# nubomedia/NUBOMEDIA-VCA

Hardware: AMD Instinct MI355X
Metric: 1080p frames/sec/node (NuboFaceDetector); achieved HBM GB/s vs peak (higher is better)
Workload: dtype i32 rect sums / f32 products / f64 stage sums (u8 pixels)

## Files before the change

nubomedia-vca_amd/csrc/api.cpp:

```cpp
#include "nvca_internal.h"
#include "plan.h"
#include "host_logic.h"
#include <cstdio>
#include <cstring>
#include <cmath>
#include <climits>
#include <algorithm>
#include <fstream>
#include <sstream>
#include <chrono>
#if defined(__SSE2__)
#include <emmintrin.h>
#endif
#include <stdexcept>
#include <new>
#include <thread>
#include <condition_variable>
#include <atomic>

using namespace nvca;

namespace nvca {

static bool alloc_log() { static const bool on = getenv("NVCA_ALLOC_LOG") != nullptr; return on; }
// ... 129 lines not shown
    t.pending.swap(later);
}
static void drain_timer(nvca_ctx *ctx)
{
    if (ctx->timer.pending.size() > 4096) drain_timer_now(ctx);
}

int api_catch(nvca_ctx *ctx) noexcept
{
    int code = NVCA_ERR_INTERNAL;
    const char *what = "unknown exception";
    char buf[160];
    try { throw; }
    catch (const std::bad_alloc &) { code = NVCA_ERR_NOMEM; what = "out of host memory (std::bad_alloc)"; }
    catch (const std::length_error &e) { code = NVCA_ERR_NOMEM; snprintf(buf, sizeof(buf), "container size limit exceeded (%s)", e.what()); what = buf; }
    catch (const std::exception &e) { snprintf(buf, sizeof(buf), "internal error: %s", e.what()); what = buf; }
    catch (...) { }
    if (ctx) {
        try { std::lock_guard<std::recursive_mutex> lk(ctx->mu); ctx->err.assign(what); } catch (...) { }
    }
    return code;
}

static Switches read_switches()
{
    Switches w;
    auto num = [](const char *name, int dflt) { const char *e = getenv(name); return e ? atoi(e) : dflt; };
    auto set = [](const char *name) { return getenv(name) != nullptr; };
    w.group_zero_copy = num("NVCA_GROUP_ZEROCOPY", 1) != 0;
    w.skip_cascade = set("NVCA_SKIP_CASCADE");
    w.host_group = set("NVCA_HOST_GROUP");
    w.band_map = num("NVCA_BAND_MAP", 0);
    w.band = num("NVCA_BAND", -1);
    w.host_profile = set("NVCA_HOST_PROFILE");
    w.sparse_ingest = num("NVCA_SPARSE_INGEST", 1) != 0;
    w.pyr_off = set("NVCA_PYR_OFF");
    if (set("NVCA_PART_STATS")) { const int n = num("NVCA_PART_STATS", 0); w.part_stats = n > 0 ? n : 8; }
    w.ingest_chunk = num("NVCA_INGEST_CHUNK", 8);
    w.stage_order = num("NVCA_STAGE_ORDER", 0) != 0;
    w.trk_fold = num("NVCA_TRK_FOLD", 1) != 0;
    w.spec_pairs = std::max(1, num("NVCA_SPEC_PAIRS", 1536));
    w.pair_max = num("NVCA_PAIR_MAX", 32);
    w.deep_stage = set("NVCA_DEEP_STAGE") ? std::max(1, num("NVCA_DEEP_STAGE", 0)) : 0;
    w.tiles = num("NVCA_TILES", 1) != 0;
    w.plan_debug = set("NVCA_PLAN_DEBUG");
    w.deep_lds = !set("NVCA_DEEP_LDS_OFF");
    w.trk_order = num("NVCA_TRK_ORDER", -1);
    w.host_threads = num("NVCA_HOST_THREADS", -1);
    w.two_lanes = num("NVCA_TWO_LANES", 1) != 0;
    w.roi = num("NVCA_ROI", 1) != 0;
    w.fb_dense = num("NVCA_FB_DENSE", 1) != 0;
    w.pre_cus = num("NVCA_PRE_CUS", 0);
    w.quiet = set("NVCA_QUIET");
    w.stamps_out = getenv("NVCA_STAMPS_OUT");
    return w;
}
const Switches &switches()
{
    static const Switches w = read_switches();
    return w;
}

static inline size_t round_up(size_t v, size_t a) { return (v + a - 1) / a * a; }
static inline int cv_round(double v)
{
    if (!(v > -2147483648.5 && v < 2147483647.5)) return INT_MIN;
// ... 271 lines not shown
    const size_t grp_stride = rec + 2;
    if (dev_group) {
        const void *old_gthr = rb.gthr.p;
        if (rb.grp.ensure((size_t)total * grp_stride * sizeof(int)) || rb.h_grp.ensure((size_t)total * grp_stride * sizeof(int)) ||
            rb.gthr.ensure((size_t)total * sizeof(int)) || rb.h_gthr.ensure((size_t)total * sizeof(int))) {
            ctx->set_error("device allocation failed for the grouping workspace"); return NVCA_ERR_NOMEM;
        }
        if (rb.gthr.p != old_gthr) rb.gthr_last.clear();
        job.d_grp = rb.grp.as<int>() + grp_stride * job.r0; job.h_grp = rb.h_grp.as<int>() + grp_stride * job.r0;
        if (rb.gthr_last.size() < (size_t)total) rb.gthr_last.resize(total, -1);
        if (memcmp(rb.gthr_last.data() + job.r0, group_thr, batch * sizeof(int)) != 0) {
            NVCA_HIP_CHECK(ctx, hipStreamSynchronize(ctx->cs()));
            memcpy(rb.h_gthr.as<int>() + job.r0, group_thr, batch * sizeof(int));
            NVCA_HIP_CHECK(ctx, hipMemcpyAsync(rb.gthr.as<int>() + job.r0, rb.h_gthr.as<int>() + job.r0, batch * sizeof(int), hipMemcpyHostToDevice, ctx->cs()));
            std::copy(group_thr, group_thr + batch, rb.gthr_last.begin() + job.r0);
        }
    }
    if (!dp.tasks.empty() && !skip_cascade) {
        CascadeArgs a;
        a.sum = ws.ln().sum.as<int>(); a.sqsum = ws.ln().sqsum.as<unsigned long long>();
        a.sum_slot = sum_slot; a.spitch = spitch;
        a.scales = dp.d_scales.as<ScaleRec>();
        a.stages = dp.d_stages.as<StageRec>(); a.strips = dp.d_strips.as<StripRec>(); a.pos = dp.d_pos.as<int>();
        a.order = dp.d_order.as<int>(); a.blocks_per_frame = dp.blocks_per_frame;
        a.tasks = dp.d_tasks.as<unsigned>(); a.ntasks = (int)dp.tasks.size();
        a.failbits = ws.ln().failbits.as<unsigned long long>(); a.vnf = ws.ln().vnf.as<double>();
        a.nstages = (int)dp.stages.size(); a.pair_policy = ctx->policy == NVCA_SUM_F32PAIR; a.stage_order = ctx->sw.stage_order ? 1 : 0; a.stage_hint = dp.d_stage_hint.as<int>(); a.stage_first = dp.d_stage_first.as<int>(); a.stage_thr = dp.d_stage_thr.as<float>(); a.spec_pairs = ctx->sw.spec_pairs; a.pair_max = std::min(32, std::max(0, ctx->sw.pair_max));
        a.deep_stage = dp.deep_stage; a.deep = ws.ln().deep.as<unsigned long long>(); a.deep_cap = deep_cap;
        a.hits = job.d_hits; a.hit_cap = cap;
        a.tiles = dp.d_tiles.as<TileRec>(); a.tile_order = dp.d_tile_order.as<int>();
        a.tile_blocks_per_frame = dp.tile_blocks_per_frame;
        a.tcoords = dp.d_tcoords.as<unsigned short>(); a.tile_lds = dp.tile_lds;
        a.nscales = (int)dp.scales.size(); a.key_sy = dp.key_sy; a.key_ss = dp.key_ss;
        a.bands = dp.d_bands.as<BandRec>(); a.band_order = dp.d_band_order.as<int>(); a.band_blocks_per_frame = dp.band_blocks_per_frame; a.batch = batch;
        { const int bm = ctx->sw.band_map; a.band_map = (bm > 0 && batch % (8 * bm) == 0) ? bm : 0; }
        a.deeprecs = dp.deeprecs.empty() ? nullptr : dp.d_deeprecs.as<DeepRec>(); a.deep_lds = dp.deep_lds;
        a.tilted = dp.needs_tilted ? ws.ln().tilted.as<int>() : nullptr;
        a.galpha = dp.tabs.empty() ? nullptr : dp.tabs[0]->d_galpha; a.gcls_first = dp.tabs.empty() ? nullptr : dp.tabs[0]->d_gcls_first;
        a.stump_based = dp.generic_stumps ? 1 : 0;
        if (dp.generic) {
            if (dp.needs_tilted && !a.tilted) { ctx->set_error("internal: tilted integral missing"); return NVCA_ERR_ARG; }
            { TimedLaunch t(ctx, NVCA_K_STAGE0); launch_generic(ctx->cs(), a, batch, 0); }
            { TimedLaunch t(ctx, NVCA_K_STRIP); launch_generic(ctx->cs(), a, batch, 1); }
        } else {
#ifdef NVCA_STAMPS
        {
            static DevBuf dbgbuf;
            a.dbg = nullptr;
            if (switches().stamps_out && !dbgbuf.ensure(64 * 16 * 64 * 8)) { a.dbg = dbgbuf.as<unsigned long long>(); (void)hipMemsetAsync(a.dbg, 0, 64 * 16 * 64 * 8, ctx->cs()); ctx->stamps = a.dbg; }
        }
#endif
        const int band_env = ctx->sw.band;
        const bool use_band = !dp.bands.empty() && (band_env >= 0 ? band_env != 0 : (long long)dp.bands.size() * batch >= 270 * kTilesPerCu);
        auto launch = [&](int which) {
            const int e = launch_cascade_sc(ctx->cs(), a, batch, which, ctx->lds_grant);
            if (e) ctx->set_error(std::string("hipFuncSetAttribute(MaxDynamicSharedMemorySize): ") + hipGetErrorString((hipError_t)e));
            return e;
        };
        if (!use_band) { TimedLaunch t(ctx, NVCA_K_STAGE0); if (launch(0)) return NVCA_ERR_HIP; }
        if (use_band) {
            TimedLaunch t(ctx, NVCA_K_BAND); if (launch(5)) return NVCA_ERR_HIP;
        } else {
            { TimedLaunch t(ctx, NVCA_K_TILE); if (launch(3)) return NVCA_ERR_HIP; }
            { TimedLaunch t(ctx, NVCA_K_STRIP); if (launch(1)) return NVCA_ERR_HIP; }
        }
        if (early_done) NVCA_HIP_CHECK(ctx, hipEventRecord(early_done, ctx->cs()));
        { TimedLaunch t(ctx, NVCA_K_DEEP); if (launch(2)) return NVCA_ERR_HIP; }
// ... 386 lines not shown
int nvca_ctx_set_hit_capacity(nvca_ctx *ctx, int cap)
try {
    if (!ctx || cap < 1 || cap > kMaxHitCap) return NVCA_ERR_ARG;
    ctx->hit_cap = cap;
    return NVCA_OK;
}
NVCA_API_CATCH(ctx)
int nvca_ctx_set_option(nvca_ctx *ctx, const char *name, int value)
try {
    NVCA_LOCK_OR_FAIL(ctx);
    if (!name) return NVCA_ERR_ARG;
    const std::string n(name);
    Switches &w = ctx->sw;
    bool replan = false;
    if (n == "band") w.band = value;
    else if (n == "band_map") w.band_map = value;
    else if (n == "group_zerocopy") w.group_zero_copy = value != 0;
    else if (n == "host_group") w.host_group = value != 0;
    else if (n == "skip_cascade") w.skip_cascade = value != 0;
    else if (n == "host_profile") w.host_profile = value != 0;
    else if (n == "sparse_ingest") w.sparse_ingest = value != 0;
    else if (n == "ingest_chunk") w.ingest_chunk = value;
    else if (n == "part_stats") w.part_stats = value;
    else if (n == "trk_order") w.trk_order = value;
    else if (n == "trk_fold") w.trk_fold = value != 0;
    else if (n == "quiet") w.quiet = value != 0;
    else if (n == "roi") w.roi = value != 0;
    else if (n == "fb_dense") w.fb_dense = value != 0;
    else if (n == "two_lanes") w.two_lanes = value != 0;
    else if (n == "host_threads") { w.host_threads = value; work_pool_destroy(ctx->pool); ctx->pool = nullptr; ctx->pool_tried = false; }
    else if (n == "pre_cus") w.pre_cus = value > 0 ? value : 0;
    else if (n == "plan_debug") w.plan_debug = value != 0;
    else if (n == "stage_order") w.stage_order = value != 0;
    else if (n == "spec_pairs") w.spec_pairs = value > 0 ? value : 1;
    else if (n == "pair_max") w.pair_max = value;
    else if (n == "pyr_off") { w.pyr_off = value != 0; replan = true; }
    else if (n == "tiles") { w.tiles = value != 0; replan = true; }
    else if (n == "deep_stage") { w.deep_stage = value > 0 ? value : 0; replan = true; }
    else if (n == "deep_lds") { w.deep_lds = value != 0; replan = true; }
    else { ctx->set_error("unknown option: " + n); return NVCA_ERR_ARG; }
    if (replan) {
        for (auto &kv : ctx->plans) if (kv.second->inflight) { ctx->set_error("a batch is in flight: collect it before changing a plan option"); return NVCA_ERR_ARG; }
        (void)hipSetDevice(ctx->device);
        NVCA_HIP_CHECK(ctx, hipDeviceSynchronize());
        ctx->plans.clear();
    }
    return NVCA_OK;
}
NVCA_API_CATCH(ctx)
int nvca_ctx_get_option(nvca_ctx *ctx, const char *name, int *value)
try {
    NVCA_LOCK_OR_FAIL(ctx);
    if (!name || !value) return NVCA_ERR_ARG;
    const std::string n(name);
    const Switches &w = ctx->sw;
    if (n == "band") *value = w.band;
    else if (n == "band_map") *value = w.band_map;
    else if (n == "group_zerocopy") *value = w.group_zero_copy;
    else if (n == "host_group") *value = w.host_group;
    else if (n == "skip_cascade") *value = w.skip_cascade;
    else if (n == "host_profile") *value = w.host_profile;
    else if (n == "sparse_ingest") *value = w.sparse_ingest;
    else if (n == "ingest_chunk") *value = w.ingest_chunk;
    else if (n == "part_stats") *value = w.part_stats;
    else if (n == "trk_order") *value = w.trk_order;
    else if (n == "trk_fold") *value = w.trk_fold;
    else if (n == "quiet") *value = w.quiet;
    else if (n == "roi") *value = w.roi;
    else if (n == "fb_dense") *value = w.fb_dense;
    else if (n == "two_lanes") *value = w.two_lanes;
    else if (n == "host_threads") *value = w.host_threads;
    else if (n == "pre_cus") *value = w.pre_cus;
    else if (n == "plan_debug") *value = w.plan_debug;
    else if (n == "stage_order") *value = w.stage_order;
    else if (n == "spec_pairs") *value = w.spec_pairs;
    else if (n == "pair_max") *value = w.pair_max;
    else if (n == "pyr_off") *value = w.pyr_off;
    else if (n == "tiles") *value = w.tiles;
    else if (n == "deep_stage") *value = w.deep_stage;
    else if (n == "deep_lds") *value = w.deep_lds;
    else { ctx->set_error("unknown option: " + n); return NVCA_ERR_ARG; }
    return NVCA_OK;
}
NVCA_API_CATCH(ctx)
int nvca_ctx_set_sum_policy(nvca_ctx *ctx, int policy)
try {
    if (!ctx || (policy != NVCA_SUM_F32PAIR && policy != NVCA_SUM_F64)) return NVCA_ERR_ARG;
    ctx->policy = policy;
    return NVCA_OK;
}
NVCA_API_CATCH(ctx)
int nvca_ctx_synchronize(nvca_ctx *ctx)
try {
    NVCA_LOCK_OR_FAIL(ctx);
    if (!ctx) return NVCA_ERR_ARG;
    NVCA_HIP_CHECK(ctx, hipStreamSynchronize(ctx->cs()));
    NVCA_HIP_CHECK(ctx, hipStreamSynchronize(ctx->lane_streams[kFaceLane2]));
    NVCA_HIP_CHECK(ctx, hipStreamSynchronize(ctx->lane_streams[kTrackerLane]));
#ifdef NVCA_STAMPS
    if (ctx->stamps && switches().stamps_out) {
        std::vector<unsigned long long> h(64 * 16 * 64);
        (void)hipMemcpy(h.data(), ctx->stamps, h.size() * 8, hipMemcpyDeviceToHost);
        if (FILE *f = fopen(switches().stamps_out, "wb")) { fwrite(h.data(), 8, h.size(), f); fclose(f); }
    }
    if (switches().stamps_out) roi_stamps_dump((std::string(switches().stamps_out) + ".roi.txt").c_str());
#endif
    return NVCA_OK;
// ... 1950 lines not shown
```

nubomedia-vca_amd/csrc/kernels_cascade.hip:

```cpp
#include "nvca_internal.h"

namespace nvca {

typedef const __attribute__((address_space(4))) TStumpRec CTStumpRec;
template <class T> __device__ __forceinline__ T load_const(const T *p)
{
    static_assert(sizeof(T) % 4 == 0, "dword records only");
    typedef const __attribute__((address_space(4))) int CInt;
    CInt *q = (CInt *)p;
    T r;
    int *d = (int *)&r;
#pragma unroll
    for (int i = 0; i < (int)(sizeof(T) / 4); i++) d[i] = q[i];
    return r;
}

__device__ __forceinline__ int ldsum(const int *__restrict__ sum, unsigned idx) { return sum[idx]; }

__device__ __forceinline__ double window_sqsum(const unsigned *__restrict__ sql, const uint8_t *__restrict__ sqh, bool lo_only,
                                               unsigned e0, unsigned e1, unsigned e2, unsigned e3)
{
    if (lo_only) return (double)(unsigned)(sql[e0] - sql[e1] - sql[e2] + sql[e3]);
    const unsigned long long q0 = ((unsigned long long)sqh[e0] << 32) | sql[e0], q1 = ((unsigned long long)sqh[e1] << 32) | sql[e1];
    const unsigned long long q2 = ((unsigned long long)sqh[e2] << 32) | sql[e2], q3 = ((unsigned long long)sqh[e3] << 32) | sql[e3];
// ... 480 lines not shown
    const int c0 = lds_u16(cm + (xx & 0xffffu)), c1 = lds_u16(cm + (xx >> 16));
    const int r0 = lds_u16(rm + (yy & 0xffffu)), r1 = lds_u16(rm + (yy >> 16));
    return lds_sample(r0, c0) - lds_sample(r0, c1) - lds_sample(r1, c0) + lds_sample(r1, c1);
}
__device__ __forceinline__ double lane_vote(unsigned cm, unsigned rm, double vnf, const LRec &f, int pair_policy)
{
    const int s0 = lane_rect(cm, rm, (unsigned)f.a.x, (unsigned)f.a.y);
    const int s1 = lane_rect(cm, rm, (unsigned)f.a.z, (unsigned)f.a.w);
    const double t = (double)__int_as_float(f.c.y) * vnf;
    const float p0 = (float)s0 * __int_as_float(f.b.z), p1 = (float)s1 * __int_as_float(f.b.w);
    double v = (double)p0;
    v += (double)p1;
    if (f.b.x) v += (double)((float)lane_rect(cm, rm, (unsigned)f.b.x, (unsigned)f.b.y) * __int_as_float(f.c.x));
    else if (pair_policy && f.b.y == 1) v = (double)(p0 + p1);
    return (double)__int_as_float(v >= t ? f.c.w : f.c.z);
}

#ifdef NVCA_STAMPS
#define NVCA_STAMP(a, tile, id) do { if (threadIdx.x == 0 && blockIdx.x < 64 && (tile) < 16 && (id) < 64 && (a).dbg) { unsigned long long t__; \
    asm volatile("s_memtime %0\n\ts_waitcnt lgkmcnt(0)" : "=s"(t__) :: "memory"); (a).dbg[((size_t)blockIdx.x * 16 + (tile)) * 64 + (id)] = t__; } } while (0)
#define NVCA_STAMP_VAL(a, tile, id, v) do { if (threadIdx.x == 0 && blockIdx.x < 64 && (tile) < 16 && (id) < 64 && (a).dbg) (a).dbg[((size_t)blockIdx.x * 16 + (tile)) * 64 + (id)] = (unsigned long long)(v); } while (0)
#else
#define NVCA_STAMP(a, tile, id) do { } while (0)
#define NVCA_STAMP_VAL(a, tile, id, v) do { } while (0)
#endif

struct TileLds {
    double *acc;
    unsigned short *q0, *winx, *winy; int *qn; double *vnf_s;
    unsigned short *cmap, *rmap; int *T; int pitchT;
    int tword;
    unsigned cmA, rmA;
};
__device__ __forceinline__ TileLds carve_tile(unsigned char *lds, const TileRec &t)
{
    TileLds L;
    L.acc = (double *)lds;
    L.q0 = (unsigned short *)(lds + kTileSlots * 8);
    L.winx = L.q0 + 2 * kTileSlots; L.winy = L.winx + kTileWin;
    L.qn = (int *)(L.winy + kTileWin);
    L.vnf_s = (double *)((unsigned char *)L.qn + 128);
    L.cmap = (unsigned short *)(L.vnf_s + kTileSlots);
    L.rmap = L.cmap + ((t.span_x + 3) & ~3);
    L.T = (int *)(L.rmap + ((t.span_y + 3) & ~3));
    L.pitchT = tile_pitch(t.ncol);
    L.tword = (int)(lds_addr(L.T) >> 2);
    L.cmA = lds_addr(L.cmap); L.rmA = lds_addr(L.rmap);
    return L;
}

struct TileCoords { int mapc, mapr, wx, wy; unsigned rowb, xcb[4]; };
__device__ __forceinline__ TileCoords tile_coords(const CascadeArgs &a, const TileRec &t, const ScaleRec &sc)
{
    const int tid = threadIdx.x, lane = tid & 63, wave = tid >> 6;
    constexpr int NW = kTileThreads / 64;
    const unsigned short *__restrict__ cl = a.tcoords + t.col_off, *__restrict__ rl = a.tcoords + t.row_off;
    TileCoords c;
    c.mapc = tid < t.ncol ? (int)cl[tid] : -1;
    c.mapr = tid < t.nrow ? (int)rl[tid] : -1;
    c.wx = tid < t.nx ? a.pos[sc.xpos_off + t.ix0 + tid] : 0;
    c.wy = (tid >= 64 && tid < 64 + t.ny) ? a.pos[sc.ypos_off + t.iy0 + tid - 64] : 0;
    const int nmine = t.nrow > wave ? (t.nrow - wave + NW - 1) / NW : 0;
    c.rowb = lane < nmine ? (unsigned)rl[wave + NW * lane] * (unsigned)sc.pitch * 4u : 0u;
#pragma unroll
    for (int k = 0; k < 4; k++) { const int q = lane + 64 * k; c.xcb[k] = 4u * (unsigned)cl[q < t.ncol ? q : t.ncol - 1]; }
    return c;
}
__device__ __forceinline__ void tile_commit(const CascadeArgs &a, const TileRec &t, const ScaleRec &sc, int slot, const TileLds &L, const TileCoords &c)
{
    const int tid = threadIdx.x, lane = tid & 63, wave = __builtin_amdgcn_readfirstlane(tid >> 6);
    constexpr int NW = kTileThreads / 64;
    const char *__restrict__ src = (const char *)(a.sum + (size_t)slot * a.sum_slot + sc.plane_off);
    const int nmine = t.nrow > wave ? (t.nrow - wave + NW - 1) / NW : 0;
    const int nk = (t.ncol + 63) >> 6;
    for (int j = 0; j < nmine; j++) {
        const unsigned rb = (unsigned)__builtin_amdgcn_readlane((int)c.rowb, j);
        const char *rowp = src + rb;
        int *dst = L.T + (wave + NW * j) * L.pitchT;
#pragma unroll
        for (int k = 0; k < 4; k++)
            if (k < nk && lane + 64 * k < t.ncol)
                __builtin_amdgcn_global_load_lds((gptr_t)(rowp + c.xcb[k]), (lptr_t)(dst + 64 * k), 4, 0, 0);
    }
    if (tid < 3) L.qn[tid] = 0;
    if (tid < t.nx) L.winx[tid] = (unsigned short)(c.wx - t.x0);
    if (tid >= 64 && tid < 64 + t.ny) L.winy[tid - 64] = (unsigned short)(c.wy - t.y0);
    if (c.mapc >= 0) L.cmap[c.mapc - t.x0] = (unsigned short)(tid * 4);
    if (c.mapr >= 0) L.rmap[c.mapr - t.y0] = (unsigned short)(L.tword + tid * L.pitchT);
}

__device__ __forceinline__ void queue_push_wave0(bool keep, int w, unsigned short *q, int *count)
{
    if (threadIdx.x >= 64) return;
    const int lane = threadIdx.x;
    const unsigned long long km = __ballot(keep);
    if (keep) q[__popcll(km & ((1ull << lane) - 1ull))] = (unsigned short)w;
    if (lane == 0) *count = __popcll(km);
}
__device__ __forceinline__ void queue_push(bool keep, int w, unsigned short *q, int *count)
{
    const int lane = threadIdx.x & 63;
    const unsigned long long km = __ballot(keep);
    if (km) {
        int wbase = 0;
        if (lane == 0) wbase = atomicAdd(count, __popcll(km));
        wbase = __shfl(wbase, 0);
        if (keep) q[wbase + __popcll(km & ((1ull << lane) - 1ull))] = (unsigned short)w;
    }
}

static constexpr int kStatStages = 6;
static constexpr int kPairMax = 32;
static_assert(7 * kPairMax <= kTileSlots && 64 + kTileRows <= kTileThreads && kTileRows <= kTileWin,
              "a round's seven accumulator rows fit the tile's accumulators; threads 64 .. 64 + kTileRows - 1 fill winy[kTileWin]");
template <bool VNF_LDS>
__device__ __forceinline__ void tile_stages(const CascadeArgs &a, const TileRec &t, const ScaleRec &sc, int slot, const TileLds &L, int ti = 0, int par = 0)
{
    const int tid = threadIdx.x, lane = tid & 63;
    const int wave = __builtin_amdgcn_readfirstlane(tid >> 6);
    const int *stat_r = L.qn + 4 + par * kStatStages;
    int *stat_w = L.qn + 4 + (par ^ 1) * kStatStages;
// ... 243 lines not shown
        const unsigned long long *rb = bits + (size_t)ry * sc.wpr;
        if (!((rb[ix >> 6] >> (ix & 63)) & 1ull)) keep = sc.adaptive ? visited(rb, ix) : true;
    }
    asm volatile("s_waitcnt vmcnt(0)" ::: "memory");
    __syncthreads();
    queue_push(keep, w, L.q0, &L.qn[0]);
    tile_stages<false>(a, t, sc, slot, L);
}

__global__ __launch_bounds__(kTileThreads, kTileWavesPerSimd) void k_band(CascadeArgs a)
{
    extern __shared__ __align__(16) unsigned char lds[];
    const int tid = threadIdx.x, lane = tid & 63;
    int bi = blockIdx.x / a.batch, slot = blockIdx.x - bi * a.batch;
    if (a.band_map) {
        const int xcd = blockIdx.x & 7, k = blockIdx.x >> 3;
        const int g = a.band_map;
        const int fi = k / (a.band_blocks_per_frame * g), r = k - fi * a.band_blocks_per_frame * g;
        bi = r / g; slot = xcd + 8 * (fi * g + (r - bi * g));
    }
    const BandRec b = load_const(a.bands + a.band_order[bi]);
    const ScaleRec &sc = a.scales[b.scale];
    const unsigned *__restrict__ sql = (const unsigned *)a.sqsum + (size_t)slot * 2 * a.sum_slot + sc.plane_off;
    const uint8_t *__restrict__ sqh = (const uint8_t *)((const unsigned *)a.sqsum + (size_t)slot * 2 * a.sum_slot + a.sum_slot) + sc.plane_off;
    const bool sq_lo_only = sc.sq32 != 0;
    const int ex0 = sc.eq[0] % sc.pitch, ey0 = sc.eq[0] / sc.pitch, ex1 = sc.eq[3] % sc.pitch, ey1 = sc.eq[3] / sc.pitch;
    const StageRec st0 = load_const(a.stages);
    const bool pair0 = a.pair_policy && (st0.flags & 1);
    static_assert(kTileSlots == kTileThreads, "one window per thread and tile");
    const int w = tid, ry = w >> 5, rx = w & 31;
    unsigned carry = 0;
    TileRec t = load_const(a.tiles + b.first_tile);
    TileCoords tc = tile_coords(a, t, sc);
    tile_prologue(a, carve_tile(lds, t));
    int oxw = 0, oyw = 0;
    if (ry < t.ny && rx < t.nx) { oxw = a.pos[sc.xpos_off + t.ix0 + rx]; oyw = a.pos[sc.ypos_off + t.iy0 + ry]; }
    for (int ti = 0; ti < b.ntiles; ti++) {
        __syncthreads();
        NVCA_STAMP(a, ti, 0);
        const TileLds L = carve_tile(lds, t);
        const bool active = ry < t.ny && rx < t.nx;
        int xw = oxw, yw = oyw;
        unsigned q0 = 0, q1 = 0, q2 = 0, q3 = 0, h0 = 0, h1 = 0, h2 = 0, h3 = 0;
        if (active) {
            xw -= t.x0; yw -= t.y0;
            const unsigned off = (unsigned)((t.y0 + yw) * sc.pitch + t.x0 + xw);
            const unsigned e0 = off + sc.eq[0], e1 = off + sc.eq[1], e2 = off + sc.eq[2], e3 = off + sc.eq[3];
            q0 = sql[e0]; q1 = sql[e1]; q2 = sql[e2]; q3 = sql[e3];
            if (!sq_lo_only) { h0 = sqh[e0]; h1 = sqh[e1]; h2 = sqh[e2]; h3 = sqh[e3]; }
        }
        NVCA_STAMP(a, ti, 1);
        tile_commit(a, t, sc, slot, L, tc);
        if (tid < kStatStages) L.qn[4 + ((ti + 1) & 1) * kStatStages + tid] = 0;
        TileRec tn = t; TileCoords tcn = tc; int nxw = 0, nyw = 0;
        if (ti + 1 < b.ntiles) {
            tn = load_const(a.tiles + b.first_tile + ti + 1);
            tcn = tile_coords(a, tn, sc);
            if (ry < tn.ny && rx < tn.nx) { nxw = a.pos[sc.xpos_off + tn.ix0 + rx]; nyw = a.pos[sc.ypos_off + tn.iy0 + ry]; }
        }
        NVCA_STAMP(a, ti, 2);
        asm volatile("s_waitcnt vmcnt(0)" ::: "memory");
        __syncthreads();
        NVCA_STAMP(a, ti, 3);
        bool pass0 = false;
        if (active) {
            const int c0 = L.cmap[xw + ex0], c1 = L.cmap[xw + ex1], r0 = L.rmap[yw + ey0], r1 = L.rmap[yw + ey1];
            const int ws = lds_sample(r0, c0) - lds_sample(r0, c1) - lds_sample(r1, c0) + lds_sample(r1, c1);
            const double mean = (double)ws * sc.inv_area;
            double vnf;
            if (sq_lo_only) vnf = (double)(unsigned)(q0 - q1 - q2 + q3);
            else vnf = (double)(((unsigned long long)h0 << 32) | q0) - (double)(((unsigned long long)h1 << 32) | q1) -
                       (double)(((unsigned long long)h2 << 32) | q2) + (double)(((unsigned long long)h3 << 32) | q3);
            vnf = vnf * sc.inv_area - mean * mean;
            vnf = vnf >= 0. ? sqrt(vnf) : 1.;
            L.vnf_s[w] = vnf;
            pass0 = tile_stage_pass(L.cmA + 2 * xw, L.rmA + 2 * yw, vnf, sc.trecs, st0, pair0);
        }
        const unsigned long long fb = __ballot(active && !pass0);
        const unsigned R = lane < 32 ? (unsigned)fb : (unsigned)(fb >> 32);
        bool keep = false;
        if (active && !((R >> rx) & 1u)) {
            if (!sc.adaptive) keep = true;
            else {
                int ones = 0;
                if (rx > 0) {
                    const unsigned mk = ~(R << (32 - rx));
                    ones = mk ? __clz((int)mk) : 32;
                    if (ones > rx) ones = rx;
                }
                const int cbit = (int)((carry >> (lane >> 5)) & 1u);
// ... 308 lines not shown
```

nubomedia-vca_amd/csrc/nvca_internal.h:

```cpp
#pragma once
#include <hip/hip_runtime.h>
#include <hip/hip_ext.h>
#include <stdint.h>
#include <string>
#include <vector>
#include <map>
#include <memory>
#include <mutex>
#include "../../include/nubovca.h"
#include "host_ranges.h"

namespace nvca {

struct HaarNode {
    int   rect[3][4];
    float weight[3];
    int   nrect;
    float threshold;
    int   left, right;
    int   tilted;
};
struct HaarClassifier { int first_node, nnodes, first_alpha; };
struct HaarStage { int first_cls, ncls; float threshold;  };

// ... 26 lines not shown
    int    plane_off;
    int    pitch;
    int    endX, endY;
    int    eq[4];
    int    xpos_off, ypos_off;
    int    sq32;
    int    task_off;
    int    wpr;
    int    adaptive;
    double inv_area;
    double factor;
    const struct TStumpRec *trecs;
    const struct GNodeRec *grecs;
    const struct LStumpRec *lrecs;
};

struct GNodeRec {
    short dx[3][4], dy[3][4];
    float w[3];
    float thr;
    int left, right;
    int flags;
    int pad;
};
static_assert(sizeof(GNodeRec) == 80, "GNodeRec layout");

struct StripRec { int scale, iy0, nrows, ix0, ncols, pad0, pad1, pad2; };
struct TileRec {
    int scale, ix0, iy0, nx, ny;
    int x0, y0;
    int ncol, nrow;
    int span_x, span_y;
    int col_off, row_off;
    int pad_t;
    int pad0, pad1;
};
struct TStumpRec {
    int x0[3], x1[3], y0[3], y1[3];
    float w[3];
    int nrect;
    double thr, a0, a1;
    int a0i, a1i;
};
static_assert(sizeof(TStumpRec) == 96, "TStumpRec layout is read dword by dword in kernels_cascade.hip");
struct alignas(16) LStumpRec {
    unsigned xx0, yy0, xx1, yy1, xx2, yy2;
    float w0, w1, w2, thr, a0, a1;
};
static_assert(sizeof(LStumpRec) == 48, "LStumpRec is read as three int4 in kernels_cascade.hip");
struct DeepRec { int col_off, ncol, row_off, nrow, span_x, span_y, pad0, pad1; };
static constexpr int kDeepMaxSide = 64;
static constexpr int kDeepMaxSpan = 1280;
struct BandRec { int scale, iy0, ny, first_tile, ntiles, pad0, pad1, pad2; };
static constexpr int kTileWin = 32;
static constexpr int kTileRows = 16;
static constexpr int kTileSlots = kTileWin * kTileRows;
static constexpr int kTileThreads = kTileSlots;
static constexpr int kTilesPerCu = 3;
static constexpr int kTileWavesPerSimd = (kTilesPerCu * kTileThreads / 64 + 3) / 4;
static constexpr int kTileLdsBudget = 52 * 1024;
static_assert(kTilesPerCu * kTileLdsBudget <= 160 * 1024 && kTilesPerCu * kTileThreads <= 32 * 64, "tile residency per CU");
static constexpr int kTileMaxCols = 256;
__host__ __device__ inline int tile_pitch(int ncol) { return ncol | 1; }
__host__ __device__ inline int tile_lds_fixed()
{
    return kTileSlots * 8 + 2 * kTileSlots * 2 + 4 * kTileWin + 128 + kTileSlots * 8;
}
__host__ __device__ inline int tile_lds_bytes(int ncol, int nrow, int span_x, int span_y)
{
    return 4 * nrow * tile_pitch(ncol) + 2 * ((span_x + 3) & ~3) + 2 * ((span_y + 3) & ~3) + tile_lds_fixed();
}

static constexpr int kStripMaxWin = 512;
static constexpr int kIntegralBand = 16;

struct ResizeTab {
    int sw = 0, sh = 0, dw = 0, dh = 0;
    int mode = 0;
    int xmax = 0;
    std::vector<int> xofs, yofs;
    std::vector<short> ialpha, ibeta;
};
void build_resize_tab(int sw, int sh, int dw, int dh, ResizeTab &t);

struct Switches {
    bool group_zero_copy = true;
    bool skip_cascade = false;
    bool host_group = false;
    int  band_map = 0;
    int  band = -1;
    bool host_profile = false;
    bool sparse_ingest = true;
    bool pyr_off = false;
    int  part_stats = 0;
    int  ingest_chunk = 8;
    int  deep_stage = 0;
    bool tiles = true;
    bool plan_debug = false;
    bool deep_lds = true;
    bool trk_fold = true;
    int  trk_order = -1;
    int  host_threads = -1;
    bool two_lanes = true;
    bool fb_dense = true;
    bool roi = true;
    bool stage_order = false;
    int  pair_max = 32;
    int  spec_pairs = 1536;
    int  pre_cus = 0;
    bool quiet = false;
    const char *stamps_out = nullptr;
};
const Switches &switches();

#define NVCA_HIP_CHECK(ctx, expr)                                                   \
    do {                                                                            \
        hipError_t e__ = (expr);                                                    \
        if (e__ != hipSuccess) {                                                    \
            (ctx)->set_error(std::string(#expr) + ": " + hipGetErrorString(e__));   \
            return NVCA_ERR_HIP;                                                    \
        }                                                                           \
    } while (0)

struct DevBuf {
    void *p = nullptr; size_t bytes = 0;
    int ensure(size_t n);
    void release();
    template <class T> T *as() const { return (T *)p; }
};
struct PinnedBuf {
    void *p = nullptr; size_t bytes = 0;
    int ensure(size_t n);
    void release();
    template <class T> T *as() const { return (T *)p; }
};

struct BounceRing {
    static constexpr size_t kSlot = 8u << 20;
    static constexpr int kSlots = 12;
    PinnedBuf buf; hipEvent_t ev[kSlots] = {}; bool pending[kSlots] = {}; int next = 0;
    void release() { for (hipEvent_t &e : ev) if (e) { (void)hipEventDestroy(e); e = nullptr; } buf.release(); }
};
// ... 176 lines not shown
                     int batch);

bool small_integral_fits(const PreGeom &g);
void launch_small_integral(hipStream_t st, const uint8_t *gray, const uint8_t *lut, int lut_stride, const PreGeom &g, int *sum,
                           unsigned long long *sqsum, int batch);

struct TrkSlot {
    const uint8_t *src;
    uint8_t *prev;
    float *mhi;
    float ts, delbound;
    float seg;
    int threshold;
    int has_prev;
    int sstride;
    int min_area;
    long long max_area;
};
struct CompAcc { int minx, miny, maxx, maxy, seed, pad; };
void launch_tracker(hipStream_t st, const void *d_slots, int batch, int w, int h, bool vec4, int *labels, void *acc,
                    int *out, int cap, bool run_ccl, uint8_t *flags, int order , int *roots, int roots_cap, int mode, int *tiles, int tick);
inline size_t tracker_count_offset(int w, int h, int batch) { return ((size_t)((w + 255) / 256) * h * batch + 63) & ~(size_t)63; }
inline size_t tracker_flag_bytes(int w, int h, int batch) { return tracker_count_offset(w, h, batch) + sizeof(int) * (size_t)batch; }

struct CascadeArgs {
    const int *sum; const unsigned long long *sqsum;
    size_t sum_slot;
    int spitch;
    const ScaleRec *scales; const StageRec *stages;
    const StripRec *strips; const int *pos;
    const int *order; int blocks_per_frame;
    const TileRec *tiles; const int *tile_order; int tile_blocks_per_frame;
    const unsigned short *tcoords; int tile_lds;
    const BandRec *bands; const int *band_order; int band_blocks_per_frame; int batch; int band_map;
    const DeepRec *deeprecs;
    int nscales;
    const unsigned *tasks; int ntasks;
    unsigned long long *failbits;
    double *vnf;
    int nstages; int pair_policy;
    int stage_order;
    int *stage_hint;
    int spec_pairs;
    int pair_max;
    const float *stage_thr;
    const int *stage_first;
    int deep_stage;
    int deep_lds;
    unsigned long long *deep;
    unsigned deep_cap;
    int key_sy, key_ss;
    unsigned long long *hits;
    unsigned hit_cap;
    const int *tilted;
    const float *galpha;
    const int *gcls_first;
    int stump_based;
#ifdef NVCA_STAMPS
    unsigned long long *dbg;
#endif
};
int launch_cascade_sc(hipStream_t st, const CascadeArgs &a, int batch, int which, int *lds_grant);
#if defined(__HIPCC__)
#define NVCA_HD __host__ __device__
#else
#define NVCA_HD
#endif
// ... 126 lines not shown
```

nubomedia-vca_amd/csrc/plan.cpp:

```cpp
#include "plan.h"
#include <cmath>
#include <cfloat>
#include <cstring>
#include <algorithm>
#include <climits>
#include <cstdlib>

namespace nvca {

static inline int cv_round(double v) { return (int)lrint(v); }
static inline int cv_floor(double v) { return (int)floor(v); }
static inline short sat_short(int v) { return (short)(v < -32768 ? -32768 : (v > 32767 ? 32767 : v)); }

void build_resize_tab(int sw, int sh, int dw, int dh, ResizeTab &t)
{
    t.sw = sw; t.sh = sh; t.dw = dw; t.dh = dh;
    t.xofs.assign(dw, 0); t.yofs.assign(dh, 0);
    t.ialpha.assign(2 * (size_t)dw, 0); t.ibeta.assign(2 * (size_t)dh, 0);
    t.xmax = dw;
    double inv_scale_x = (double)dw / sw, inv_scale_y = (double)dh / sh;
    double scale_x = 1. / inv_scale_x, scale_y = 1. / inv_scale_y;
    int iscale_x = cv_round(scale_x), iscale_y = cv_round(scale_y);
    bool is_area_fast = std::fabs(scale_x - iscale_x) < DBL_EPSILON && std::fabs(scale_y - iscale_y) < DBL_EPSILON;
    if (sw == dw && sh == dh) { t.mode = 0; return; }
// ... 203 lines not shown
    return 8 * maxlen;
}

bool DetectPlan::hit_valid(unsigned key) const
{
    const size_t s = key >> key_ss, iy = (key >> key_sy) & ((1u << (key_ss - key_sy)) - 1u), ix = key & ((1u << key_sy) - 1u);
    return s < specs.size() && ix < specs[s].xs.size() && iy < specs[s].ys.size();
}

nvca_rect DetectPlan::hit_rect(unsigned key) const
{
    const int s = key >> key_ss, iy = (key >> key_sy) & ((1u << (key_ss - key_sy)) - 1u), ix = key & ((1u << key_sy) - 1u);
    const ScaleSpec &sp = specs[s];
    const int x = sp.xs[ix], y = sp.ys[iy];
    if (sp.out_factor != 0) return nvca_rect{cv_round(x * sp.out_factor), cv_round(y * sp.out_factor), sp.out_w, sp.out_h};
    return nvca_rect{x, y, sp.out_w, sp.out_h};
}

int DetectPlan::build_custom(nvca_ctx *ctx, const Cascade &c, std::vector<ScaleSpec> &&in, bool allow_tiles, std::string &err)
{
    specs = std::move(in);
    const int ns = (int)c.stages.size();
    if (ctx->sw.deep_stage > 0) { deep_stage = ctx->sw.deep_stage; return build_tables(ctx, c, allow_tiles, err); }
    if (!ctx->sw.tiles || c.generic()) { deep_stage = 6; return build_tables(ctx, c, allow_tiles, err); }
    deep_stage = ns;
    int rc = build_tables(ctx, c, allow_tiles, err);
    if (rc == NVCA_OK && !generic && ctx->sw.tiles && ns > 6 && (!strips.empty() || (min_tile_side > 0 && min_tile_side < std::min(max_tile_side, 20)))) {
        deep_stage = 6;
        rc = build_tables(ctx, c, allow_tiles, err);
    }
    return rc;
}

int DetectPlan::build_tables(nvca_ctx *ctx, const Cascade &c, bool allow_tiles, std::string &err)
{
    generic = c.generic(); needs_tilted = c.has_tilted; generic_stumps = c.stump_based;
    nstumps = (int)c.cls.size();
    scales.clear(); strips.clear(); pos.clear(); tasks.clear(); tiles.clear(); release_tables();
    min_tile_side = 0; max_tile_side = 0;
    bool use_tiles = ctx->sw.tiles;
    if (generic) use_tiles = false;
    (void)allow_tiles;
    tcoords.clear(); tile_lds = 0; bands.clear(); band_order.clear(); band_blocks_per_frame = 0;
    {
        auto bits = [](size_t n) { int b = 1; while ((1ull << b) < n) b++; return b; };
        size_t mx = 1, my = 1;
        for (const ScaleSpec &sp : specs) { mx = std::max(mx, sp.xs.size()); my = std::max(my, sp.ys.size()); }
        const int bx = bits(mx), by = bits(my), bs = bits(std::max<size_t>(specs.size(), 1));
        if (bx + by + bs > 32 || specs.size() > 4095) { err = "scan too large for the candidate key (scales x rows x columns of windows beyond 2^32)"; return NVCA_ERR_ARG; }
        key_sy = bx; key_ss = bx + by;
    }
    if (c.stage_rec_cache.empty()) {
        std::vector<StageRec> tmp; build_stage_recs(c, tmp);
        c.stage_rec_cache.resize(tmp.size() * sizeof(StageRec));
        if (!tmp.empty()) memcpy(c.stage_rec_cache.data(), tmp.data(), c.stage_rec_cache.size());
    }
    stages.resize(c.stage_rec_cache.size() / sizeof(StageRec));
    if (!stages.empty()) memcpy(stages.data(), c.stage_rec_cache.data(), c.stage_rec_cache.size());
    stage_first.clear();
    for (const StageRec &sr : stages) stage_first.push_back(sr.first);
    stage_first.push_back(stages.empty() ? 0 : stages.back().first + stages.back().count);
    stage_first.insert(stage_first.end(), 8, INT_MAX);
    stage_thr.clear();
    for (const StageRec &sr : stages) stage_thr.push_back(sr.thr);
    stage_thr.insert(stage_thr.end(), 8, 0.f);
    std::vector<long long> strip_w, tile_w;
// ... 69 lines not shown
                     tile_lds_bytes(worst_c, worst_r, worst_sx, worst_sy) <= kTileLdsBudget;
                if (ok) {
                    if (ctx->sw.plan_debug)
                        fprintf(stderr, "[nvca plan] scale %zu factor %.3f windows %d x %d: tile side %d, %d x %d samples, %d B of LDS (budget %d)\n", s, sp.table_factor > 0 ? sp.table_factor : sp.out_factor,
                                sr.endX, sr.endY, tw, worst_c, worst_r, tile_lds_bytes(worst_c, worst_r, worst_sx, worst_sy), kTileLdsBudget);
                    break;
                }
            }
            if (tw >= 1) {
                min_tile_side = min_tile_side ? std::min(min_tile_side, tw) : tw; max_tile_side = max_tile;
                const int th = std::min(tw, kTileRows);
                for (int iy0 = 0; iy0 < sr.endY; iy0 += th) {
                    coords(yp, iy0, std::min(iy0 + th, sr.endY), offy, cy);
                    BandRec b; memset(&b, 0, sizeof(b));
                    b.scale = (int)s; b.iy0 = iy0; b.ny = std::min(th, sr.endY - iy0); b.first_tile = (int)tiles.size();
                    b.ntiles = (sr.endX + tw - 1) / tw;
                    bands.push_back(b);
                    const int row_off = (int)tcoords.size();
                    for (int v : cy) tcoords.push_back((unsigned short)v);
                    for (int ix0 = 0; ix0 < sr.endX; ix0 += tw) {
                        coords(xp, ix0, std::min(ix0 + tw, sr.endX), offx, cx);
                        TileRec t; memset(&t, 0, sizeof(t));
                        t.scale = (int)s; t.ix0 = ix0; t.iy0 = iy0;
                        t.nx = std::min(tw, sr.endX - ix0); t.ny = std::min(th, sr.endY - iy0);
                        t.x0 = xp[ix0]; t.y0 = yp[iy0];
                        t.ncol = (int)cx.size(); t.nrow = (int)cy.size();
                        t.span_x = cx.back() - t.x0 + 1; t.span_y = cy.back() - t.y0 + 1;
                        t.col_off = (int)tcoords.size(); t.row_off = row_off;
                        for (int v : cx) tcoords.push_back((unsigned short)v);
                        tile_lds = std::max(tile_lds, tile_lds_bytes(t.ncol, t.nrow, t.span_x, t.span_y));
                        tiles.push_back(t);
                        tile_w.push_back((long long)t.nx * t.ny + 256);
                    }
                }
            } else tw = 0;
        }
        if (!tw) {
            if (sr.endX <= kStripMaxWin) {
                const int rows_per = std::max(1, std::min(kStripMaxWin / sr.endX, 64));
                for (int iy = 0; iy < sr.endY; iy += rows_per) {
                    StripRec st; memset(&st, 0, sizeof(st));
                    st.scale = (int)s; st.iy0 = iy; st.nrows = std::min(rows_per, sr.endY - iy); st.ix0 = 0; st.ncols = sr.endX;
                    strips.push_back(st);
                    strip_w.push_back((long long)st.nrows * st.ncols);
                }
            } else {
                const int nseg = (sr.endX + kStripMaxWin - 1) / kStripMaxWin, seg = (sr.endX + nseg - 1) / nseg;
                for (int iy = 0; iy < sr.endY; iy++)
                    for (int x0 = 0; x0 < sr.endX; x0 += seg) {
                        StripRec st; memset(&st, 0, sizeof(st));
                        st.scale = (int)s; st.iy0 = iy; st.nrows = 1; st.ix0 = x0; st.ncols = std::min(seg, sr.endX - x0);
                        strips.push_back(st);
                        strip_w.push_back((long long)st.ncols);
                    }
            }
        }
    }
    blocks_per_frame = build_xcd_order(strip_w, order);
    tile_blocks_per_frame = build_xcd_order(tile_w, tile_order);
    if (!strips.empty()) bands.clear();
    if (!strips.empty() && use_tiles && !generic && !ctx->sw.quiet) {
        static bool noted = false;
        if (!noted) {
            noted = true;
            fprintf(stderr, "nubovca: a scan (%d x %d image, %zu scales) does not fit the LDS tile kernels and runs on the row-strip fallback (k_strip): same results, slower; NVCA_PLAN_DEBUG=1 prints the per-scale tile sizes (this note is printed once)\n",
                    cols, rows, specs.size());
// ... 127 lines not shown
```

Measured before the change: 20540.

## Reuse overlapping integral-image columns across band tiles with an LDS ring buffer

Adds a ring-buffer mode for band-scheduled tiles. Integral-image columns already loaded into LDS by the previous tile in the same band are kept, and each new tile fetches only the columns it adds, at ring positions planned on the host. The goal is to cut redundant global loads of overlapping tile columns. In exchange it adds planner complexity, wraparound address handling in the commit, and possibly a larger LDS footprint per band, which could lower occupancy.

Result: no change. 20360, median of 2 (-0.9%).

```diff
diff --git a/nubomedia-vca_amd/csrc/api.cpp b/nubomedia-vca_amd/csrc/api.cpp
--- a/nubomedia-vca_amd/csrc/api.cpp
+++ b/nubomedia-vca_amd/csrc/api.cpp
@@ -185,6 +185,7 @@
     w.host_group = set("NVCA_HOST_GROUP");
     w.band_map = num("NVCA_BAND_MAP", 0);
     w.band = num("NVCA_BAND", -1);
+    w.band_ring = num("NVCA_BAND_RING", 1) != 0;
     w.host_profile = set("NVCA_HOST_PROFILE");
     w.sparse_ingest = num("NVCA_SPARSE_INGEST", 1) != 0;
     w.pyr_off = set("NVCA_PYR_OFF");
@@ -522,7 +523,7 @@
         a.tile_blocks_per_frame = dp.tile_blocks_per_frame;
         a.tcoords = dp.d_tcoords.as<unsigned short>(); a.tile_lds = dp.tile_lds;
         a.nscales = (int)dp.scales.size(); a.key_sy = dp.key_sy; a.key_ss = dp.key_ss;
-        a.bands = dp.d_bands.as<BandRec>(); a.band_order = dp.d_band_order.as<int>(); a.band_blocks_per_frame = dp.band_blocks_per_frame; a.batch = batch;
+        a.bands = dp.d_bands.as<BandRec>(); a.band_order = dp.d_band_order.as<int>(); a.band_blocks_per_frame = dp.band_blocks_per_frame; a.batch = batch; a.band_ring = ctx->sw.band_ring ? 1 : 0;
         { const int bm = ctx->sw.band_map; a.band_map = (bm > 0 && batch % (8 * bm) == 0) ? bm : 0; }
         a.deeprecs = dp.deeprecs.empty() ? nullptr : dp.d_deeprecs.as<DeepRec>(); a.deep_lds = dp.deep_lds;
         a.tilted = dp.needs_tilted ? ws.ln().tilted.as<int>() : nullptr;
@@ -975,6 +976,7 @@
     else if (n == "pre_cus") w.pre_cus = value > 0 ? value : 0;
     else if (n == "plan_debug") w.plan_debug = value != 0;
     else if (n == "stage_order") w.stage_order = value != 0;
+    else if (n == "band_ring") w.band_ring = value != 0;
     else if (n == "spec_pairs") w.spec_pairs = value > 0 ? value : 1;
     else if (n == "pair_max") w.pair_max = value;
     else if (n == "pyr_off") { w.pyr_off = value != 0; replan = true; }
@@ -1016,6 +1018,7 @@
     else if (n == "pre_cus") *value = w.pre_cus;
     else if (n == "plan_debug") *value = w.plan_debug;
     else if (n == "stage_order") *value = w.stage_order;
+    else if (n == "band_ring") *value = w.band_ring;
     else if (n == "spec_pairs") *value = w.spec_pairs;
     else if (n == "pair_max") *value = w.pair_max;
     else if (n == "pyr_off") *value = w.pyr_off;
diff --git a/nubomedia-vca_amd/csrc/kernels_cascade.hip b/nubomedia-vca_amd/csrc/kernels_cascade.hip
--- a/nubomedia-vca_amd/csrc/kernels_cascade.hip
+++ b/nubomedia-vca_amd/csrc/kernels_cascade.hip
@@ -536,7 +536,7 @@
     int tword;
     unsigned cmA, rmA;
 };
-__device__ __forceinline__ TileLds carve_tile(unsigned char *lds, const TileRec &t)
+__device__ __forceinline__ TileLds carve_tile(unsigned char *lds, int ncol, int span_x, int span_y)
 {
     TileLds L;
     L.acc = (double *)lds;
@@ -545,13 +545,15 @@
     L.qn = (int *)(L.winy + kTileWin);
     L.vnf_s = (double *)((unsigned char *)L.qn + 128);
     L.cmap = (unsigned short *)(L.vnf_s + kTileSlots);
-    L.rmap = L.cmap + ((t.span_x + 3) & ~3);
-    L.T = (int *)(L.rmap + ((t.span_y + 3) & ~3));
-    L.pitchT = tile_pitch(t.ncol);
+    L.rmap = L.cmap + ((span_x + 3) & ~3);
+    L.T = (int *)(L.rmap + ((span_y + 3) & ~3));
+    L.pitchT = tile_pitch(ncol);
     L.tword = (int)(lds_addr(L.T) >> 2);
     L.cmA = lds_addr(L.cmap); L.rmA = lds_addr(L.rmap);
     return L;
 }
+__device__ __forceinline__ TileLds carve_tile(unsigned char *lds, const TileRec &t) { return carve_tile(lds, t.ncol, t.span_x, t.span_y); }
+__device__ __forceinline__ TileLds carve_ring(unsigned char *lds, const BandRec &b, const TileRec &t) { return carve_tile(lds, b.ring_cap, b.ring_span, t.span_y); }
 
 struct TileCoords { int mapc, mapr, wx, wy; unsigned rowb, xcb[4]; };
 __device__ __forceinline__ TileCoords tile_coords(const CascadeArgs &a, const TileRec &t, const ScaleRec &sc)
@@ -591,6 +593,59 @@
     if (tid >= 64 && tid < 64 + t.ny) L.winy[tid - 64] = (unsigned short)(c.wy - t.y0);
     if (c.mapc >= 0) L.cmap[c.mapc - t.x0] = (unsigned short)(tid * 4);
     if (c.mapr >= 0) L.rmap[c.mapr - t.y0] = (unsigned short)(L.tword + tid * L.pitchT);
+}
+
+__device__ __forceinline__ TileCoords ring_coords(const CascadeArgs &a, const TileRec &t, const ScaleRec &sc, unsigned rowb)
+{
+    const int tid = threadIdx.x, lane = tid & 63;
+    const unsigned short *__restrict__ cl = a.tcoords + t.col_off;
+    TileCoords c;
+    c.mapc = tid < t.ncol ? (int)cl[tid] : -1;
+    c.mapr = tid < t.ncol ? (int)cl[t.ncol + tid] : 0;
+    c.wx = tid < t.nx ? a.pos[sc.xpos_off + t.ix0 + tid] : 0;
+    c.wy = (tid >= 64 && tid < 64 + t.ny) ? a.pos[sc.ypos_off + t.iy0 + tid - 64] : 0;
+    c.rowb = rowb;
+#pragma unroll
+    for (int k = 0; k < 4; k++) { const int q = lane + 64 * k; c.xcb[k] = q < t.ring_nnew ? 4u * (unsigned)cl[2 * t.ncol + q] : 0u; }
+    return c;
+}
+__device__ __forceinline__ void ring_rows(const TileRec &t, const TileLds &L, const TileCoords &c)
+{
+    if (c.mapr >= 0) L.rmap[c.mapr - t.y0] = (unsigned short)(L.tword + threadIdx.x * L.pitchT);
+}
+__device__ __forceinline__ void ring_commit(const CascadeArgs &a, const TileRec &t, int cap, const ScaleRec &sc, int slot, const TileLds &L, const TileCoords &c)
+{
+    const int tid = threadIdx.x, lane = tid & 63, wave = __builtin_amdgcn_readfirstlane(tid >> 6);
+    constexpr int NW = kTileThreads / 64;
+    const char *__restrict__ src = (const char *)(a.sum + (size_t)slot * a.sum_slot + sc.plane_off);
+    const int nmine = t.nrow > wave ? (t.nrow - wave + NW - 1) / NW : 0;
+    const int nnew = t.ring_nnew, nk = (nnew + 63) >> 6;
+    const int qw = cap - t.ring_s0;
+    unsigned xw = 0;
+    if (qw < nnew && (qw & 63)) {
+#pragma unroll
+        for (int k = 0; k < 4; k++)
+            if (k == (qw >> 6)) xw = (unsigned)__shfl((int)c.xcb[k], (lane + (qw & 63)) & 63);
+    }
+    for (int j = 0; j < nmine; j++) {
+        const unsigned rb = (unsigned)__builtin_amdgcn_readlane((int)c.rowb, j);
+        const char *rowp = src + rb;
+        int *dst = L.T + (wave + NW * j) * L.pitchT;
+#pragma unroll
+        for (int k = 0; k < 4; k++) {
+            if (k < nk) {
+                int s = t.ring_s0 + 64 * k;
+                if (s >= cap) s -= cap;
+                const int nact = min(64, nnew - 64 * k), n1 = min(nact, cap - s);
+                if (lane < n1) __builtin_amdgcn_global_load_lds((gptr_t)(rowp + c.xcb[k]), (lptr_t)(dst + s), 4, 0, 0);
+                if (lane < nact - n1) __builtin_amdgcn_global_load_lds((gptr_t)(rowp + xw), (lptr_t)dst, 4, 0, 0);
+            }
+        }
+    }
+    if (tid < 3) L.qn[tid] = 0;
+    if (tid < t.nx) L.winx[tid] = (unsigned short)(c.wx - t.x0);
+    if (tid >= 64 && tid < 64 + t.ny) L.winy[tid - 64] = (unsigned short)(c.wy - t.y0);
+    if (c.mapc >= 0) L.cmap[c.mapc - t.x0] = (unsigned short)c.mapr;
 }
 
 __device__ __forceinline__ void queue_push_wave0(bool keep, int w, unsigned short *q, int *count)
@@ -900,13 +955,18 @@
     unsigned carry = 0;
     TileRec t = load_const(a.tiles + b.first_tile);
     TileCoords tc = tile_coords(a, t, sc);
+    const bool ring = a.band_ring && b.ring_cap > 0;
+    if (ring) {
+        ring_rows(t, carve_ring(lds, b, t), tc);
+        tc = ring_coords(a, t, sc, tc.rowb);
+    }
     tile_prologue(a, carve_tile(lds, t));
     int oxw = 0, oyw = 0;
     if (ry < t.ny && rx < t.nx) { oxw = a.pos[sc.xpos_off + t.ix0 + rx]; oyw = a.pos[sc.ypos_off + t.iy0 + ry]; }
     for (int ti = 0; ti < b.ntiles; ti++) {
         __syncthreads();
         NVCA_STAMP(a, ti, 0);
-        const TileLds L = carve_tile(lds, t);
+        const TileLds L = ring ? carve_ring(lds, b, t) : carve_tile(lds, t);
         const bool active = ry < t.ny && rx < t.nx;
         int xw = oxw, yw = oyw;
         unsigned q0 = 0, q1 = 0, q2 = 0, q3 = 0, h0 = 0, h1 = 0, h2 = 0, h3 = 0;
@@ -918,12 +978,13 @@
             if (!sq_lo_only) { h0 = sqh[e0]; h1 = sqh[e1]; h2 = sqh[e2]; h3 = sqh[e3]; }
         }
         NVCA_STAMP(a, ti, 1);
-        tile_commit(a, t, sc, slot, L, tc);
+        if (ring) ring_commit(a, t, b.ring_cap, sc, slot, L, tc);
+        else tile_commit(a, t, sc, slot, L, tc);
         if (tid < kStatStages) L.qn[4 + ((ti + 1) & 1) * kStatStages + tid] = 0;
         TileRec tn = t; TileCoords tcn = tc; int nxw = 0, nyw = 0;
         if (ti + 1 < b.ntiles) {
             tn = load_const(a.tiles + b.first_tile + ti + 1);
-            tcn = tile_coords(a, tn, sc);
+            tcn = ring ? ring_coords(a, tn, sc, tc.rowb) : tile_coords(a, tn, sc);
             if (ry < tn.ny && rx < tn.nx) { nxw = a.pos[sc.xpos_off + tn.ix0 + rx]; nyw = a.pos[sc.ypos_off + tn.iy0 + ry]; }
         }
         NVCA_STAMP(a, ti, 2);
diff --git a/nubomedia-vca_amd/csrc/nvca_internal.h b/nubomedia-vca_amd/csrc/nvca_internal.h
--- a/nubomedia-vca_amd/csrc/nvca_internal.h
+++ b/nubomedia-vca_amd/csrc/nvca_internal.h
@@ -82,8 +82,8 @@
     int ncol, nrow;
     int span_x, span_y;
     int col_off, row_off;
-    int pad_t;
-    int pad0, pad1;
+    int ring_s0, ring_nnew;
+    int pad1;
 };
 struct TStumpRec {
     int x0[3], x1[3], y0[3], y1[3];
@@ -101,7 +101,7 @@
 struct DeepRec { int col_off, ncol, row_off, nrow, span_x, span_y, pad0, pad1; };
 static constexpr int kDeepMaxSide = 64;
 static constexpr int kDeepMaxSpan = 1280;
-struct BandRec { int scale, iy0, ny, first_tile, ntiles, pad0, pad1, pad2; };
+struct BandRec { int scale, iy0, ny, first_tile, ntiles, ring_cap, ring_span, pad0; };
 static constexpr int kTileWin = 32;
 static constexpr int kTileRows = 16;
 static constexpr int kTileSlots = kTileWin * kTileRows;
@@ -158,6 +158,7 @@
     int  pair_max = 32;
     int  spec_pairs = 1536;
     int  pre_cus = 0;
+    bool band_ring = true;
     bool quiet = false;
     const char *stamps_out = nullptr;
 };
@@ -400,7 +401,7 @@
     const int *order; int blocks_per_frame;
     const TileRec *tiles; const int *tile_order; int tile_blocks_per_frame;
     const unsigned short *tcoords; int tile_lds;
-    const BandRec *bands; const int *band_order; int band_blocks_per_frame; int batch; int band_map;
+    const BandRec *bands; const int *band_order; int band_blocks_per_frame; int batch; int band_map; int band_ring;
     const DeepRec *deeprecs;
     int nscales;
     const unsigned *tasks; int ntasks;
diff --git a/nubomedia-vca_amd/csrc/plan.cpp b/nubomedia-vca_amd/csrc/plan.cpp
--- a/nubomedia-vca_amd/csrc/plan.cpp
+++ b/nubomedia-vca_amd/csrc/plan.cpp
@@ -259,6 +259,44 @@
     return rc;
 }
 
+static int plan_band_ring(BandRec &b, std::vector<TileRec> &tiles, std::vector<unsigned short> &tcoords)
+{
+    b.ring_cap = 0; b.ring_span = 0;
+    TileRec *tb = &tiles[b.first_tile];
+    const int nrow = tb[0].nrow, span_y = tb[0].span_y;
+    for (int i = 1; i < b.ntiles; i++)
+        if (tb[i].row_off != tb[0].row_off || tb[i].nrow != nrow || tb[i].span_y != span_y || tb[i].y0 != tb[0].y0) return 0;
+    std::vector<int> U, idx;
+    int lo = INT_MAX, hi = 0;
+    for (int i = 0; i < b.ntiles; i++) { lo = std::min<int>(lo, tcoords[tb[i].col_off]); hi = std::max<int>(hi, tcoords[tb[i].col_off + tb[i].ncol - 1]); }
+    idx.assign(hi - lo + 1, -1);
+    int cap = 0, span = 0, prev_first = 0;
+    std::vector<int> nnew(b.ntiles), newb(b.ntiles);
+    for (int i = 0; i < b.ntiles; i++) {
+        const TileRec &t = tb[i];
+        newb[i] = (int)U.size();
+        for (int j = 0; j < t.ncol; j++) { const int c = tcoords[t.col_off + j]; if (idx[c - lo] < 0) { idx[c - lo] = (int)U.size(); U.push_back(c); } }
+        nnew[i] = (int)U.size() - newb[i];
+        int first = INT_MAX;
+        for (int j = 0; j < t.ncol; j++) first = std::min(first, idx[tcoords[t.col_off + j] - lo]);
+        if (first < prev_first || nnew[i] > kTileMaxCols) return 0;
+        cap = std::max(cap, (int)U.size() - first); span = std::max(span, t.span_x);
+        prev_first = first;
+    }
+    const int bytes = tile_lds_bytes(cap, nrow, span, span_y);
+    if (bytes > kTileLdsBudget || nrow * tile_pitch(cap) >= 65536) return 0;
+    b.ring_cap = cap; b.ring_span = span;
+    for (int i = 0; i < b.ntiles; i++) {
+        TileRec &t = tb[i];
+        const int off = (int)tcoords.size();
+        for (int j = 0; j < t.ncol; j++) tcoords.push_back(tcoords[t.col_off + j]);
+        for (int j = 0; j < t.ncol; j++) tcoords.push_back((unsigned short)(idx[tcoords[t.col_off + j] - lo] % cap * 4));
+        for (int j = 0; j < nnew[i]; j++) tcoords.push_back((unsigned short)U[newb[i] + j]);
+        t.col_off = off; t.ring_s0 = newb[i] % cap; t.ring_nnew = nnew[i];
+    }
+    return bytes;
+}
+
 int DetectPlan::build_tables(nvca_ctx *ctx, const Cascade &c, bool allow_tiles, std::string &err)
 {
     generic = c.generic(); needs_tilted = c.has_tilted; generic_stumps = c.stump_based;
@@ -394,6 +432,7 @@
                         tiles.push_back(t);
                         tile_w.push_back((long long)t.nx * t.ny + 256);
                     }
+                    tile_lds = std::max(tile_lds, plan_band_ring(bands.back(), tiles, tcoords));
                 }
             } else tw = 0;
         }
```
